# pengzhangzhi/ab_opt

Hardware: AMD Instinct MI355X
Metric: denoising steps/sec (256-res complex, 100-step sampler) (higher is better)
Workload: dtype f32

## Files before the change

### ab_opt_amd/csrc/ipa_core.hip

```cpp
#include <cstdlib>
#include "tail_common.h"
#include "kernels.h"

namespace abopt {

constexpr int NPW = 8, RPW = BI / NPW;
constexpr int NTH = 1024;
constexpr int SROW = 16 * JC + 4;
constexpr int SCLD = 17;
constexpr float kLog2e = 1.4426950408889634f;
constexpr float kSqrt13 = 0.5773502691896258f;
constexpr float kScale2 = kSqrt13 * kLog2e;
constexpr float kMask2 = 1e5f * kLog2e;
constexpr int SPLIT_ROW = H * C + H * D + H * P * 3;

__device__ __forceinline__ int sp_off(int h, int kq) { return h * JC + 4 * ((kq + (h >> 1)) & 3); }

__device__ __forceinline__ void point_local(float dx, float dy, float dz, float r0, float r1, float r2, float r3, float r4, float r5, float r6, float r7,
                                            float r8, float& lx, float& ly, float& lz, float& d, float& inv) {
    lx = __builtin_fmaf(r6, dz, __builtin_fmaf(r3, dy, r0 * dx));
    ly = __builtin_fmaf(r7, dz, __builtin_fmaf(r4, dy, r1 * dx));
    lz = __builtin_fmaf(r8, dz, __builtin_fmaf(r5, dy, r2 * dx));
    d = sqrtf(__builtin_fmaf(lz, lz, __builtin_fmaf(ly, ly, lx * lx)));
    inv = 1.f / (d + 1e-4f);
// ... 450 lines not shown
        sv_ += ringb[SLOT];                                                                                              \
        sv_ *= kScale2;                                                                                                  \
        float l2_[4];                                                                                                    \
        _Pragma("unroll") for (int r_ = 0; r_ < 4; ++r_) {                                                               \
            const float x_ = sv_[r_];                                                                                    \
            l2_[r_] = ((mk4_ >> (8 * r_)) & 0xffu) ? x_ : x_ - kMask2;                                                   \
        }                                                                                                                \
        const float mx_ = rows_max(fmaxf(fmaxf(l2_[0], l2_[1]), fmaxf(l2_[2], l2_[3])));                                 \
        const float mn_ = fmaxf(m_run[II], mx_);                                                                         \
        const float sc_ = __builtin_amdgcn_exp2f(m_run[II] - mn_);                                                       \
        f32x4 pv_;                                                                                                       \
        _Pragma("unroll") for (int r_ = 0; r_ < 4; ++r_) pv_[r_] = __builtin_amdgcn_exp2f(l2_[r_] - mn_);                \
        const float ps_ = rows_sum((pv_[0] + pv_[1]) + (pv_[2] + pv_[3]));                                               \
        l_run[II] = l_run[II] * sc_ + ps_;                                                                               \
        m_run[II] = mn_;                                                                                                 \
        _Pragma("unroll") for (int mt_ = 0; mt_ < 4; ++mt_) accP[II][mt_] *= sc_;                                        \
        _Pragma("unroll") for (int r_ = 0; r_ < 4; ++r_)                                                                 \
            _Pragma("unroll") for (int mt_ = 0; mt_ < 4; ++mt_) accP[II][mt_] = mfma4(ring[SLOT][r_][mt_], pv_[r_], accP[II][mt_]); \
        *reinterpret_cast<f32x4*>(spp_) = pv_;                                                                           \
        if (kq == 0) scl[((PAR) * BI + il_) * SCLD + fm] = sc_;                                                          \
    }
#define PP_CHUNK(K, CH, PAR)                                                                                             \
    {                                                                                                                    \
        const uint32_t mk4_ = *reinterpret_cast<const uint32_t*>(&mkc[(CH) * JC + kq * 4]);                              \
        PP_POS((2 * (K)) % 3, 0, CH, K, PAR)                                                                             \
        PP_POS((2 * (K) + 1) % 3, 1, CH, K, PAR)                                                                         \
    }
        int c = 0, j = 0;
        const uint8_t* mkc = mk;
        bool mi_b[RPW];
        auto block_begin = [&]() {
            if (j > 0) {
                bk = blk(j);
#pragma unroll
                for (int ii = 0; ii < RPW; ++ii) { zrow[ii] = zrow_n[ii]; pbrow[ii] = pbrow_n[ii]; }
            }
            has_next = j + 1 < nb;
            { const PBlk bn = blk(j + 1); rows_of(bn, zrow_n, pbrow_n); }
            mkc = mk + (j & 1) * mkld;
#pragma unroll
            for (int ii = 0; ii < RPW; ++ii) {
                mi_b[ii] = (bk.i0 + il0 + ii < L) && mkc[min(bk.i0 + il0 + ii, L - 1)] != 0;
                m_run[ii] = -INFINITY; l_run[ii] = 0.f;
#pragma unroll
                for (int mt = 0; mt < 4; ++mt) accP[ii][mt] = (f32x4){0.f, 0.f, 0.f, 0.f};
            }
        };
        auto block_end = [&]() {
#pragma unroll
            for (int ii = 0; ii < RPW; ++ii) {
                const int il = il0 + ii, i = bk.i0 + il;
                if (kq == 0) lsum[il * SCLD + fm] = l_run[ii];
                if (i < L && fm < H) {
                    const float inv = mi_b[ii] ? 1.f / l_run[ii] : 0.f;
                    float* fo = feat + (bk.rowbase + i) * FEAT + fm * C + kq * 16;
#pragma unroll
                    for (int r = 0; r < 4; ++r)
                        reinterpret_cast<f32x4*>(fo)[r] = (f32x4){accP[ii][0][r] * inv, accP[ii][1][r] * inv, accP[ii][2][r] * inv, accP[ii][3][r] * inv};
                }
            }
        };
#define PP_STEP(K, G)                                                                                                    \
    {                                                                                                                    \
        if (c == 0) block_begin();                                                                                       \
        PP_CHUNK(K, c, (G) & 1)                                                                                          \
        if (c == nchunk - 1) { block_end(); c = 0; ++j; } else ++c;                                                      \
        __syncthreads();                                                                                \
    }
        int g = 0;
        for (; g + 3 <= gtot; g += 3) { PP_STEP(0, g) PP_STEP(1, g + 1) PP_STEP(2, g + 2) }
        if (g < gtot) {
            PP_STEP(0, g)
            if (g + 1 < gtot) PP_STEP(1, g + 1)
        }
#undef PP_STEP
        __syncthreads();
    } else if (wave < NPW + 4) {
        const int h0 = (wave - NPW) * 3;
        const int atid = tid - NPW * 64;
        f32x4 kf[3][4];
        auto kv_of = [&](const PBlk& b) { return reinterpret_cast<const f32x4*>(kvfrag) + (int64_t)b.n * nchunk * H * 512; };
#define PA_ISSUE(HH, KV, CH) { const f32x4* fr_ = (KV) + ((int64_t)(CH) * H + h0 + (HH)) * 512 + lane;                   \
        _Pragma("unroll") for (int s_ = 0; s_ < 4; ++s_) kf[HH][s_] = fr_[s_ * 64]; }
        auto produce = [&](int buf, const f32x4* kv_next, int ch_next) {
#pragma unroll
            for (int hh = 0; hh < 3; ++hh) {
                const int h = h0 + hh;
                const f32x4* qh = qf + (h * 4) * 64 + lane;
                const f32x4 q0 = qh[0], q1 = qh[64], q2 = qh[128], q3 = qh[192];
                f32x4 acc0 = (f32x4){0.f, 0.f, 0.f, 0.f}, acc1 = acc0;
#pragma unroll
                for (int s = 0; s < 4; ++s) { acc0 = mfma4(kf[hh][0][s], q0[s], acc0); acc1 = mfma4(kf[hh][2][s], q2[s], acc1); }
#pragma unroll
                for (int s = 0; s < 4; ++s) { acc0 = mfma4(kf[hh][1][s], q1[s], acc0); if (s < 3) acc1 = mfma4(kf[hh][3][s], q3[s], acc1); }
                const f32x4 sres = acc0 + acc1;
                if (hh == 0) PA_ISSUE(0, kv_next, ch_next) else if (hh == 1) PA_ISSUE(1, kv_next, ch_next) else PA_ISSUE(2, kv_next, ch_next)
                *reinterpret_cast<f32x4*>(sp + (buf * BI + fm) * SROW + sp_off(h, kq)) = sres;
                __builtin_amdgcn_sched_barrier(0);
            }
        };
        auto kv_pos = [&](int p, const f32x4*& kv, int& ch) {
            const int pc = min(p, gtot - 1);
            const PBlk b = blk(pc / nchunk);
            kv = kv_of(b); ch = pc % nchunk;
        };
        {
            const f32x4* kv0; int ch0;
            kv_pos(0, kv0, ch0);
            PA_ISSUE(0, kv0, ch0) PA_ISSUE(1, kv0, ch0) PA_ISSUE(2, kv0, ch0)
        }
        fill_first();
        __syncthreads();
        { const f32x4* kv1; int ch1; kv_pos(1, kv1, ch1); produce(0, kv1, ch1); }
        __syncthreads();
        int bufn = 1;
        for (int g = 0; g < gtot; ++g) {
            const int gn = g + 1;
            if (gn < gtot) {
                if (gn % nchunk == 0) {
                    const int jn = gn / nchunk;
                    const PBlk bnx = blk(jn);
                    const f32x4* qg = reinterpret_cast<const f32x4*>(qfrag) + ((int64_t)bnx.n * nib + bnx.i0 / BI) * (H * 4 * 64);
#pragma unroll
                    for (int hh = 0; hh < 3; ++hh) {
                        f32x4 tq[4];
#pragma unroll
                        for (int s_ = 0; s_ < 4; ++s_) tq[s_] = qg[((h0 + hh) * 4 + s_) * 64 + lane];
#pragma unroll
                        for (int s_ = 0; s_ < 4; ++s_) qf[((h0 + hh) * 4 + s_) * 64 + lane] = tq[s_];
                    }
                    uint8_t* mkn = mk + (jn & 1) * mkld;
                    for (int e = atid; e < mkld; e += 4 * 64) mkn[e] = (e < L) ? mask[bnx.rowbase + e] : 0;
                    wave_lds_sync();
                }
                const f32x4* kvx; int chx;
                kv_pos(gn + 1, kvx, chx);
                produce(bufn, kvx, chx);
                bufn = (bufn == 2) ? 0 : bufn + 1;
            }
            if (g >= nchunk && g % nchunk == 1) {
                const PBlk bp = blk(g / nchunk - 1);
                persist_point_epilogue(ptsb, R, t, feat, bp.rowbase, bp.i0, L, atid, 4 * 64);
            }
            __syncthreads();
        }
        __syncthreads();
        { const PBlk bl = blk(nb - 1); persist_point_epilogue(ptsb, R, t, feat, bl.rowbase, bl.i0, L, atid, 4 * 64); }
    } else {
        const int h0 = (wave - NPW - 4) * 3;
        f32x4 vf[3][4];
        f32x4 accV[3][2], accT[3][2];
#pragma unroll
        for (int hh = 0; hh < 3; ++hh)
#pragma unroll
            for (int k = 0; k < 2; ++k) { accV[hh][k] = (f32x4){0.f, 0.f, 0.f, 0.f}; accT[hh][k] = (f32x4){0.f, 0.f, 0.f, 0.f}; }
        auto kv_of = [&](const PBlk& b) { return reinterpret_cast<const f32x4*>(kvfrag) + (int64_t)b.n * nchunk * H * 512; };
#define PC_ISSUE(HH, KV, CH) { const f32x4* fr_ = (KV) + ((int64_t)(CH) * H + h0 + (HH)) * 512 + 4 * 64 + lane;         \
        _Pragma("unroll") for (int s_ = 0; s_ < 4; ++s_) vf[HH][s_] = fr_[s_ * 64]; }
        auto kv_pos = [&](int p, const f32x4*& kv, int& ch) {
            const int pc = min(p, gtot - 1);
            const PBlk b = blk(pc / nchunk);
            kv = kv_of(b); ch = pc % nchunk;
        };
        auto consume = [&](int buf, int par, const f32x4* kv_next, int ch_next) {
#pragma unroll
            for (int hh = 0; hh < 3; ++hh) {
                const int h = h0 + hh;
                const float sc = scl[(par * BI + fm) * SCLD + h];
                const f32x4 pa = *reinterpret_cast<const f32x4*>(sp + (buf * BI + fm) * SROW + sp_off(h, kq));
                accV[hh][0] *= sc; accV[hh][1] *= sc; accT[hh][0] *= sc; accT[hh][1] *= sc;
#pragma unroll
                for (int s = 0; s < 4; ++s) {
                    accV[hh][0] = mfma4(vf[hh][s][0], pa[s], accV[hh][0]);
                    accV[hh][1] = mfma4(vf[hh][s][1], pa[s], accV[hh][1]);
                    accT[hh][0] = mfma4(vf[hh][s][2], pa[s], accT[hh][0]);
                    accT[hh][1] = mfma4(vf[hh][s][3], pa[s], accT[hh][1]);
                }
                if (hh == 0) PC_ISSUE(0, kv_next, ch_next) else if (hh == 1) PC_ISSUE(1, kv_next, ch_next) else PC_ISSUE(2, kv_next, ch_next)
                __builtin_amdgcn_sched_barrier(0);
            }
        };
        auto block_epilogue = [&](int j) {
            const PBlk b = blk(j);
            const uint8_t* mkc = mk + (j & 1) * mkld;
            const bool mi_c = (b.i0 + fm < L) && mkc[min(b.i0 + fm, L - 1)] != 0;
            const int i = b.i0 + fm;
#pragma unroll
            for (int hh = 0; hh < 3; ++hh) {
                const int h = h0 + hh;
                const float inv = mi_c ? 1.f / lsum[fm * SCLD + h] : 0.f;
                if (i < L) {
                    float* fo = feat + (b.rowbase + i) * FEAT + H * C + h * D + kq * 4;
                    *reinterpret_cast<f32x4*>(fo) = accV[hh][0] * inv;
                    *reinterpret_cast<f32x4*>(fo + 16) = accV[hh][1] * inv;
                }
                float* po = ptsb + (fm * H + h) * (P * 3) + kq * 3;
#pragma unroll
                for (int r = 0; r < 3; ++r) { po[r] = accT[hh][0][r] * inv; po[12 + r] = accT[hh][1][r] * inv; }
#pragma unroll
                for (int k = 0; k < 2; ++k) { accV[hh][k] = (f32x4){0.f, 0.f, 0.f, 0.f}; accT[hh][k] = (f32x4){0.f, 0.f, 0.f, 0.f}; }
            }
        };
        {
            const f32x4* kv0; int ch0;
            kv_pos(0, kv0, ch0);
            PC_ISSUE(0, kv0, ch0) PC_ISSUE(1, kv0, ch0) PC_ISSUE(2, kv0, ch0)
        }
        fill_first();
        __syncthreads();
        __syncthreads();
        __syncthreads();
        int buf = 0;
        for (int g = 1; g <= gtot; ++g) {
            const int p = g - 1;
            const f32x4* kvx; int chx;
            kv_pos(g, kvx, chx);
            consume(buf, p & 1, kvx, chx);
            buf = (buf == 2) ? 0 : buf + 1;
            if (p % nchunk == nchunk - 1) block_epilogue(p / nchunk);
            __syncthreads();
        }
    }
#undef PP_ISSUE
#undef PP_POS
#undef PP_CHUNK
#undef PA_ISSUE
#undef PC_ISSUE
}

constexpr int BI2 = 32, NPW2 = 4, RPW2 = BI2 / NPW2, NTH2 = 512, HPW = 6;

#define C32_L2(x, r) __builtin_fmaf((x), kScale2, mterm_[r])
__device__ long long g_clock_probe[2];
constexpr int PROF_SLOTS = 2048;
__device__ unsigned long long g_prof_span[PROF_SLOTS][2];
__global__ void prof_span_reset_kernel() {
    const int i = blockIdx.x * 256 + threadIdx.x;
    if (i < PROF_SLOTS) { g_prof_span[i][0] = ~0ull; g_prof_span[i][1] = 0ull; }
}
struct TailArgs {
    const float *wot, *wmf, *x, *ubias, *g1, *be1, *b0, *b1, *b2, *g2, *be2;
    float* out;
    unsigned* xt;
};
constexpr int C32_LOOP_LDS_FLOATS = 3 * 32 * SROW + 2 * 32 * SCLD + 32 * SCLD + 32 * 32;
constexpr int C32F_PTS_OFF = ((C32_LOOP_LDS_FLOATS * 4 + 2048 + 255) / 256) * 256;
constexpr int C32F_PTSLD = H * P * 3 + 4;
constexpr int C32F_LDS_BYTES = C32F_PTS_OFF + 32 * C32F_PTSLD * 4;
constexpr int C32F_U_OFF = 0, C32F_YS_OFF = MR * XLD * 4, C32F_APA_OFF = 2 * MR * XLD * 4;
constexpr int C32F_BIAS_OFF = 2 * OT_STAGE;
static_assert(2 * OT_STAGE <= 3 * 32 * SROW * 4, "staging buffers must fit into the S/P tile");
static_assert(C32F_BIAS_OFF + 3 * F * 4 <= 3 * 32 * SROW * 4 && C32F_APA_OFF + OT_NT * AP_PLANE <= 2 * OT_STAGE && OT_NT * AP_PLANE <= 32 * C32F_PTSLD * 4, "phase-2 buffers of the fused tail");
static_assert(C32F_LDS_BYTES <= 160 * 1024, "LDS of the fused block kernel");

__device__ __forceinline__ float mul_rn(float a, float b) {
#pragma clang fp contract(off)
    return a * b;
}
__device__ __forceinline__ void stage_put4(char* buf, int row, int col, float v0, float v1, float v2, float v3) {
    unsigned h0, l0, h1, l1;
    split_pair2(v0, v1, h0, l0);
    split_pair2(v2, v3, h1, l1);
    char* d = buf + row * OT_SROW + col * 2;
    *reinterpret_cast<uint2*>(d) = make_uint2(h0, h1);
    *reinterpret_cast<uint2*>(d + OT_PLANE) = make_uint2(l0, l1);
}

template <bool FUSE, bool ZT>
__global__ __launch_bounds__(NTH2) void ipa_core32_kernel(const float* __restrict__ qfrag, const float* __restrict__ kvfrag, const float* __restrict__ z,
                                                          const uint8_t* __restrict__ mask, const float* __restrict__ R, const float* __restrict__ t,
                                                          float* __restrict__ feat, const float* __restrict__ pbc, int L, int nib2, int xcd_remap, int z_shared,
                                                          TailArgs ta, int prof_slot, const float* __restrict__ zt, const float* __restrict__ zsc) {
    extern __shared__ __attribute__((aligned(16))) char smem_raw[];
    float* sp = reinterpret_cast<float*>(smem_raw);
    float* scl = sp + 3 * BI2 * SROW;
    float* lsum = scl + 2 * BI2 * SCLD;
    float* mlr = lsum + BI2 * SCLD;
    uint8_t* mk = reinterpret_cast<uint8_t*>(mlr + BI2 * 32);
    int n, ib;
    {
        const int b = blockIdx.x;
        if (xcd_remap == 2) {
            const int xcd = b & 7, k = b >> 3, per = nib2 * z_shared, r = k % per;
            ib = r / z_shared; n = (xcd + 8 * (k / per)) * z_shared + r % z_shared;
        } else if (xcd_remap) { const int xcd = b & 7, k = b >> 3; n = xcd + 8 * (k / nib2); ib = k % nib2; }
        else { n = b / nib2; ib = b % nib2; }
    }
    const int tid = threadIdx.x, lane = tid & 63, fm = lane & 15, kq = lane >> 4;
    const int wave = __builtin_amdgcn_readfirstlane(tid >> 6);
    const int nchunk = (L + JC - 1) / JC, nib16 = (L + BI - 1) / BI;
    const long long probe_c0 = clock64(), probe_w0 = wall_clock64();
    if (prof_slot >= 0 && threadIdx.x == 0) atomicMin(&g_prof_span[prof_slot][0], (unsigned long long)probe_w0);
    const int i0 = ib * BI2;
    const int64_t rowbase = (int64_t)n * L;
    const int64_t zbase = z_shared ? (int64_t)(n / z_shared) * L : rowbase;
    auto fill_mask = [&]() { for (int e = tid; e < nchunk * JC; e += NTH2) mk[e] = (e < L) ? mask[rowbase + e] : 0; };
    char* const stage = smem_raw;
    float* const ptsf = reinterpret_cast<float*>(smem_raw + C32F_PTS_OFF);
    const int64_t row0f = rowbase + i0, row_endf = rowbase + L;
    TailP2Pre<NTH2 / 64> pre;
    constexpr int RD = 12;
    struct WT { u32x4 h, l; };
    auto consumer = [&](int cb, WT (&wt)[RD]) {
        const u32x4* wfr = reinterpret_cast<const u32x4*>(ta.wot) + (int64_t)cb * OT_ST * OT_WVEC + lane;
        auto kstep = [&](int i) { return min(ot_chunk_at(min(i / OT_SPC, OT_NCH - 1)) * OT_SPC + (i % OT_SPC), OT_ST - 1); };
        f32x16 acc[4];
#pragma unroll
        for (int g = 0; g < 4; ++g) acc_zero(acc[g]);
        __syncthreads();
        const char* xrd = stage + (lane & 31) * OT_SROW + (lane >> 5) * 16;
#define C32F_KSTEP(P_, KK, NK)                                                                                           \
        {                                                                                                                \
            const int i_ = (P_) * OT_SPC + (KK);                                                                         \
            const u32x4 wH = wt[(KK) % RD].h, wL = wt[(KK) % RD].l;                                                      \
            const u32x4 xh = xnh, xl = xnl;                                                                              \
            if ((KK) + 1 < (NK)) {                                                                                       \
                xnh = *reinterpret_cast<const u32x4*>(xb + ((KK) % OT_SPC + 1) * 32); xnl = *reinterpret_cast<const u32x4*>(xb + ((KK) % OT_SPC + 1) * 32 + OT_PLANE); \
            }                                                                                                            \
            ot_kstep3(wH, wL, xh, xl, acc[((KK) % OT_SPC) / OT_SPW]);                                                    \
            if (i_ + RD < OT_ST) { const u32x4* nf_ = wfr + (int64_t)kstep(i_ + RD) * OT_WVEC; wt[(KK) % RD].h = nf_[0]; wt[(KK) % RD].l = nf_[64]; } \
        }
#define C32F_XFIRST() { xnh = *reinterpret_cast<const u32x4*>(xb); xnl = *reinterpret_cast<const u32x4*>(xb + OT_PLANE); }
        u32x4 xnh, xnl;
        static_assert(OT_SPC == 12 && OT_ST - (OT_NCH - 1) * OT_SPC == 6 && ot_chunk_at(OT_NCH - 1) == OT_NCH - 1, "positions 0..8 are full chunks, the last one holds six k-steps");
        static_assert((2 * OT_SPC) % RD == 0, "ring slots must repeat every two positions");
        for (int p = 0; p < OT_NCH - 2; p += 2) {
            {
                const char* xb = xrd;
                C32F_XFIRST()
                C32F_KSTEP(p, 0, 12) C32F_KSTEP(p, 1, 12) C32F_KSTEP(p, 2, 12) C32F_KSTEP(p, 3, 12) C32F_KSTEP(p, 4, 12) C32F_KSTEP(p, 5, 12)
                C32F_KSTEP(p, 6, 12) C32F_KSTEP(p, 7, 12) C32F_KSTEP(p, 8, 12) C32F_KSTEP(p, 9, 12) C32F_KSTEP(p, 10, 12) C32F_KSTEP(p, 11, 12)
                __syncthreads();
            }
            {
                const char* xb = xrd + OT_STAGE;
                C32F_XFIRST()
                C32F_KSTEP(p, 12, 24) C32F_KSTEP(p, 13, 24) C32F_KSTEP(p, 14, 24) C32F_KSTEP(p, 15, 24) C32F_KSTEP(p, 16, 24) C32F_KSTEP(p, 17, 24)
                C32F_KSTEP(p, 18, 24) C32F_KSTEP(p, 19, 24) C32F_KSTEP(p, 20, 24) C32F_KSTEP(p, 21, 24) C32F_KSTEP(p, 22, 24) C32F_KSTEP(p, 23, 24)
                __syncthreads();
            }
        }
        {
            const char* xb = xrd;
            C32F_XFIRST()
            C32F_KSTEP(8, 0, 12) C32F_KSTEP(8, 1, 12) C32F_KSTEP(8, 2, 12) C32F_KSTEP(8, 3, 12) C32F_KSTEP(8, 4, 12) C32F_KSTEP(8, 5, 12)
            C32F_KSTEP(8, 6, 12) C32F_KSTEP(8, 7, 12) C32F_KSTEP(8, 8, 12) C32F_KSTEP(8, 9, 12) C32F_KSTEP(8, 10, 12) C32F_KSTEP(8, 11, 12)
            __syncthreads();
        }
        {
            const char* xb = xrd + OT_STAGE;
            C32F_XFIRST()

            C32F_KSTEP(8, 12, 18) C32F_KSTEP(8, 13, 18) C32F_KSTEP(8, 14, 18) C32F_KSTEP(8, 15, 18) C32F_KSTEP(8, 16, 18) C32F_KSTEP(8, 17, 18)
            __syncthreads();
        }
#undef C32F_KSTEP
#undef C32F_XFIRST
        float (*us)[XLD] = reinterpret_cast<float (*)[XLD]>(smem_raw + C32F_U_OFF);
#pragma unroll
        for (int g = 0; g < 4; ++g) {
            f32x4 v;
#pragma unroll
            for (int e = 0; e < 4; ++e) {
                const int q = 4 * g + e;
                v[e] = (acc[0][q] + acc[1][q]) + (acc[2][q] + acc[3][q]);
            }
            *reinterpret_cast<f32x4*>(&us[lane & 31][cb * 32 + g * 8 + (lane >> 5) * 4]) = v;
        }
    };
    auto consumer_prefetch = [&](int cb, WT (&wt)[RD]) {
        const u32x4* wfr = reinterpret_cast<const u32x4*>(ta.wot) + (int64_t)cb * OT_ST * OT_WVEC + lane;
#pragma unroll
        for (int j = 0; j < RD; ++j) { const u32x4* f = wfr + (int64_t)(ot_chunk_at(0) * OT_SPC + j) * OT_WVEC; wt[j].h = f[0]; wt[j].l = f[64]; }
        static_assert(RD <= OT_SPC, "the first fragments belong to position 0");
    };

    if (wave < NPW2) {
        const int il0 = wave * RPW2;
        const int rows_tot_ = ((int)gridDim.x / nib2 / (z_shared ? z_shared : 1)) * L;
        const __amdgpu_buffer_rsrc_t zrs = ZT ? __builtin_amdgcn_make_buffer_rsrc(const_cast<float*>(zt), 0, (unsigned)rows_tot_ * (unsigned)nchunk * (JC * C * 4), 0x00020000)
                                              : __builtin_amdgcn_make_buffer_rsrc(const_cast<float*>(z + zbase * (int64_t)L * C), 0, L * L * C * 4, 0x00020000);
        const __amdgpu_buffer_rsrc_t brs = __builtin_amdgcn_make_buffer_rsrc(const_cast<float*>(pbc), 0, (unsigned)rows_tot_ * (unsigned)nchunk * (H * JC * 4), 0x00020000);
        int zrow[RPW2], pbrow[RPW2];
#pragma unroll
        for (int ii = 0; ii < RPW2; ++ii) {
            const int row = min(i0 + il0 + ii, L - 1);
            zrow[ii] = ZT ? ((int)zbase + row) * (JC * C * 4) : row * L * (C * 4);
            pbrow[ii] = ((int)zbase + row) * (H * JC * 4);
        }
        const unsigned lane_b = (unsigned)fm * 16u;
        const unsigned pb_lane = (unsigned)(min(fm, H - 1) * JC + kq * 4) * 4u;
        f32x4 ring[3][4], ringb[4];
        unsigned koff_[4], boff_;
#define P2_KOFF(CH)                                                                                                      \
    {                                                                                                                    \
        const int ch_ = min((CH), nchunk - 1);                                        \
        _Pragma("unroll") for (int r_ = 0; r_ < 4; ++r_) koff_[r_] = ZT ? ((unsigned)ch_ * (unsigned)(rows_tot_ * (JC * C * 4)) + (unsigned)(r_ * 1024 + lane * 16)) : (unsigned)min(ch_ * JC + kq * 4 + r_, L - 1) * (unsigned)(C * 4) + lane_b; \
    }
#define P2_BOFF(CH) boff_ = (unsigned)min((CH), nchunk - 1) * ((unsigned)rows_tot_ * (unsigned)(H * JC * 4)) + pb_lane;
#define P2_ISSUE_Z(SLOT, II)                                                                                            \
        _Pragma("unroll") for (int r_ = 0; r_ < 4; ++r_)                                                                \
            ring[SLOT][r_] = __builtin_bit_cast(f32x4, __builtin_amdgcn_raw_buffer_load_b128(zrs, koff_[r_], zrow[II], 2));
#define P2_ISSUE_B(SLOT, II) ringb[SLOT] = __builtin_bit_cast(f32x4, __builtin_amdgcn_raw_buffer_load_b128(brs, boff_, pbrow[II], 2));
        P2_KOFF(0) P2_BOFF(0)
        P2_ISSUE_B(0, 0) P2_ISSUE_Z(0, 0) P2_ISSUE_B(1, 1) P2_ISSUE_Z(1, 1) P2_ISSUE_B(2, 2)
        fill_mask();
        f32x4 accP[RPW2][4];
        float* mlw = mlr + (il0 * 16 + fm) * 2;
#pragma unroll
        for (int ii = 0; ii < RPW2; ++ii) {
            if (kq == 0) *reinterpret_cast<float2*>(mlw + ii * 32) = make_float2(-INFINITY, 0.f);
#pragma unroll
            for (int mt = 0; mt < 4; ++mt) accP[ii][mt] = (f32x4){0.f, 0.f, 0.f, 0.f};
        }
        const int spo = sp_off(fm, kq);
        __syncthreads();
        __syncthreads();
#define P2_SM(II, BUF)                                                                                                   \
    {                                                                                                                    \
        const int il_ = il0 + (II);                                                                                      \
        float* spp_ = sp + ((BUF) * BI2 + il_) * SROW + spo;                                                             \
        f32x4 sv_ = *reinterpret_cast<const f32x4*>(spp_);                                                               \
        const float2 ml_ = *reinterpret_cast<const float2*>(mlw + (II) * 32);                                            \
        sv_ += ringb[(II) & 3];                                                                                          \
        float l2_[4];                                                                                                    \
        _Pragma("unroll") for (int r_ = 0; r_ < 4; ++r_) l2_[r_] = C32_L2(sv_[r_], r_);          \
        const float mx_ = rows_max(fmaxf(fmaxf(l2_[0], l2_[1]), fmaxf(l2_[2], l2_[3])));                                 \
        const float mn_ = fmaxf(ml_.x, mx_);                                                                             \
        scn_ = __builtin_amdgcn_exp2f(ml_.x - mn_);                                                                      \
        _Pragma("unroll") for (int r_ = 0; r_ < 4; ++r_) pvn_[r_] = __builtin_amdgcn_exp2f(l2_[r_] - mn_);               \
        const float ps_ = rows_sum((pvn_[0] + pvn_[1]) + (pvn_[2] + pvn_[3]));                                           \
        const float ln_ = ml_.y * scn_ + ps_;                                                                            \
        *reinterpret_cast<f32x4*>(spp_) = pvn_;                                                                          \
        if (kq == 0) { scl[((CHPAR) * BI2 + il_) * SCLD + fm] = scn_; *reinterpret_cast<float2*>(mlw + (II) * 32) = make_float2(mn_, ln_); } \
    }
#define P2_MF(SLOT, II, K_)                                                                                              \
        accP[II][(K_) & 3] = mfma4(ring[SLOT][(K_) >> 2][(K_) & 3], pvc_[(K_) >> 2], accP[II][(K_) & 3]);                \
        __builtin_amdgcn_sched_barrier(0);
#define P2_POS(SLOT, II, CH, BUF)                                                                                        \
    {                                                                                                                    \
        const f32x4 pvc_ = pvn_;                                                                                         \
        if ((II) + 3 == 8) P2_BOFF((CH) + 1)                                 \
        if ((II) + 2 == 8) P2_KOFF((CH) + 1)                                                                             \
        P2_ISSUE_B(((II) + 3) & 3, ((II) + 3) & 7)                                                                       \
        P2_ISSUE_Z(((SLOT) + 2) % 3, ((II) + 2) & 7)                                                                     \
        const int il_ = il0 + (II) + 1;                                                                                  \
        float* spp_ = sp + ((BUF) * BI2 + il_) * SROW + spo;                                                             \
        f32x4 sv_ = *reinterpret_cast<const f32x4*>(spp_);                                                               \
        const float2 ml_ = *reinterpret_cast<const float2*>(mlw + ((II) + 1) * 32);                                      \
        __builtin_amdgcn_sched_barrier(0);                                                                               \
        P2_MF(SLOT, II, 0) P2_MF(SLOT, II, 1)                                                                            \
        sv_ += ringb[((II) + 1) & 3];                                                                                    \
        P2_MF(SLOT, II, 2)                                                                                               \
        float l2_[4];                                                                                                    \
        _Pragma("unroll") for (int r_ = 0; r_ < 4; ++r_) l2_[r_] = C32_L2(sv_[r_], r_);          \
        P2_MF(SLOT, II, 3)                                                                                               \
        float mx_ = fmaxf(fmaxf(l2_[0], l2_[1]), fmaxf(l2_[2], l2_[3]));                                                 \
        { auto a_ = __builtin_amdgcn_permlane16_swap(__float_as_uint(mx_), __float_as_uint(mx_), false, false);          \
          mx_ = fmaxf(__uint_as_float(a_[0]), __uint_as_float(a_[1])); }                                                 \
        P2_MF(SLOT, II, 4)                                                                                               \
        { auto b_ = __builtin_amdgcn_permlane32_swap(__float_as_uint(mx_), __float_as_uint(mx_), false, false);          \
          mx_ = fmaxf(__uint_as_float(b_[0]), __uint_as_float(b_[1])); }                                                 \
        const float mn_ = fmaxf(ml_.x, mx_);                                                                             \
        scn_ = __builtin_amdgcn_exp2f(ml_.x - mn_);                                                                      \
        P2_MF(SLOT, II, 5)                                                                                               \
        pvn_[0] = __builtin_amdgcn_exp2f(l2_[0] - mn_); pvn_[1] = __builtin_amdgcn_exp2f(l2_[1] - mn_); \
        P2_MF(SLOT, II, 6)                                                                                               \
        pvn_[2] = __builtin_amdgcn_exp2f(l2_[2] - mn_); pvn_[3] = __builtin_amdgcn_exp2f(l2_[3] - mn_); \
        float ps_ = (pvn_[0] + pvn_[1]) + (pvn_[2] + pvn_[3]);                                                           \
        P2_MF(SLOT, II, 7)                                                                                               \
        { auto a_ = __builtin_amdgcn_permlane16_swap(__float_as_uint(ps_), __float_as_uint(ps_), false, false);          \
          ps_ = __uint_as_float(a_[0]) + __uint_as_float(a_[1]); }                                                       \
        P2_MF(SLOT, II, 8)                                                                                               \
        { auto b_ = __builtin_amdgcn_permlane32_swap(__float_as_uint(ps_), __float_as_uint(ps_), false, false);          \
          ps_ = __uint_as_float(b_[0]) + __uint_as_float(b_[1]); }                                                       \
        const float ln_ = ml_.y * scn_ + ps_;                                                                            \
        P2_MF(SLOT, II, 9)                                                                                               \
        *reinterpret_cast<f32x4*>(spp_) = pvn_;                                                                          \
        P2_MF(SLOT, II, 10)                                                                                              \
        if (kq == 0) { scl[((CHPAR) * BI2 + il_) * SCLD + fm] = scn_; *reinterpret_cast<float2*>(mlw + ((II) + 1) * 32) = make_float2(mn_, ln_); } \
        __builtin_amdgcn_sched_barrier(0);                                                                               \
        P2_MF(SLOT, II, 11)                                                                                              \
        accP[(II) + 1][0] *= scn_;                                                                                       \
        P2_MF(SLOT, II, 12)                                                                                              \
        accP[(II) + 1][1] *= scn_;                                                                                       \
        P2_MF(SLOT, II, 13)                                                                                              \
        accP[(II) + 1][2] *= scn_;                                                                                       \
        P2_MF(SLOT, II, 14)                                                                                              \
        accP[(II) + 1][3] *= scn_;                                                                                       \
        P2_MF(SLOT, II, 15)                                                                                              \
    }
#define P2_POS_LAST(SLOT, II, CH)                                                                                        \
    {                                                                                                                    \
        const f32x4 pvc_ = pvn_;                                                                                         \
        if ((II) + 3 == 8) P2_BOFF((CH) + 1)                                 \
        if ((II) + 2 == 8) P2_KOFF((CH) + 1)                                                                             \
        P2_ISSUE_B(((II) + 3) & 3, ((II) + 3) & 7)                                                                       \
        P2_ISSUE_Z(((SLOT) + 2) % 3, ((II) + 2) & 7)                                                                     \
        _Pragma("unroll") for (int r_ = 0; r_ < 4; ++r_)                                                                 \
            _Pragma("unroll") for (int mt_ = 0; mt_ < 4; ++mt_) accP[II][mt_] = mfma4(ring[SLOT][r_][mt_], pvc_[r_], accP[II][mt_]); \
        __builtin_amdgcn_sched_barrier(0);                                                                               \
    }
#define P2H_SPLIT()                                                                                                      \
        { unsigned h01_, l01_, h23_, l23_;                                                                               \
          split_pair2(pvn_[0] * 16384.f, pvn_[1] * 16384.f, h01_, l01_); split_pair2(pvn_[2] * 16384.f, pvn_[3] * 16384.f, h23_, l23_); \
          pkn_ = (u32x4){h01_, h23_, l01_, l23_}; }
#define P2H_SM(II, BUF)                                                                                                   \
    {                                                                                                                    \
        const int il_ = il0 + (II);                                                                                      \
        float* spp_ = sp + ((BUF) * BI2 + il_) * SROW + spo;                                                             \
        f32x4 sv_ = *reinterpret_cast<const f32x4*>(spp_);                                                               \
        const float2 ml_ = *reinterpret_cast<const float2*>(mlw + (II) * 32);                                            \
        sv_ += ringb[(II) & 3];                                                                                          \
        float l2_[4];                                                                                                    \
        _Pragma("unroll") for (int r_ = 0; r_ < 4; ++r_) l2_[r_] = C32_L2(sv_[r_], r_);                                  \
        const float mx_ = rows_max(fmaxf(fmaxf(l2_[0], l2_[1]), fmaxf(l2_[2], l2_[3])));                                 \
        const float mn_ = fmaxf(ml_.x, mx_);                                                                             \
        scn_ = __builtin_amdgcn_exp2f(ml_.x - mn_);                                                                      \
        f32x4 pvn_;                                                                                                      \
        _Pragma("unroll") for (int r_ = 0; r_ < 4; ++r_) pvn_[r_] = __builtin_amdgcn_exp2f(l2_[r_] - mn_);               \
        const float ps_ = rows_sum((pvn_[0] + pvn_[1]) + (pvn_[2] + pvn_[3]));                                           \
        const float ln_ = ml_.y * scn_ + ps_;                                                                            \
        P2H_SPLIT()                                                                                                      \
        *reinterpret_cast<f32x4*>(spp_) = pvn_;                               \
        if (kq == 0) { scl[((CHPAR) * BI2 + il_) * SCLD + fm] = scn_; *reinterpret_cast<float2*>(mlw + (II) * 32) = make_float2(mn_, ln_); } \
    }
#define P2H_MF(SLOT, II, K_)                                                                                              \
        { const u32x4 za_ = __builtin_bit_cast(u32x4, ring[SLOT][(K_) & 3]);                                              \
          if ((K_) >> 2) accP[II][(K_) & 3] = mfma_h16((u32x2){za_[0], za_[1]}, bl_, accP[II][(K_) & 3]);                 \
          else accP[II][(K_) & 3] = mfma_h(za_, bh_, accP[II][(K_) & 3]); }                                              \
        __builtin_amdgcn_sched_barrier(0);
#define P2H_POS(SLOT, II, CH, BUF)                                                                                        \
    {                                                                                                                    \
        const u32x4 bh_ = (u32x4){pkn_[0], pkn_[1], pkn_[0], pkn_[1]}; const u32x2 bl_ = (u32x2){pkn_[2], pkn_[3]};          \
        if ((II) + 3 == 8) P2_BOFF((CH) + 1)                                 \
        if ((II) + 2 == 8) P2_KOFF((CH) + 1)                                                                             \
        P2_ISSUE_B(((II) + 3) & 3, ((II) + 3) & 7)                                                                       \
        P2_ISSUE_Z(((SLOT) + 2) % 3, ((II) + 2) & 7)                                                                     \
        const int il_ = il0 + (II) + 1;                                                                                  \
        float* spp_ = sp + ((BUF) * BI2 + il_) * SROW + spo;                                                             \
        f32x4 sv_ = *reinterpret_cast<const f32x4*>(spp_);                                                               \
        const float2 ml_ = *reinterpret_cast<const float2*>(mlw + ((II) + 1) * 32);                                      \
        __builtin_amdgcn_sched_barrier(0);                                                                               \
        P2H_MF(SLOT, II, 0) P2H_MF(SLOT, II, 1)                                                                            \
        sv_ += ringb[((II) + 1) & 3];                                                                                    \
        float l2_[4];                                                                                                    \
        _Pragma("unroll") for (int r_ = 0; r_ < 4; ++r_) l2_[r_] = C32_L2(sv_[r_], r_);                                  \
        P2H_MF(SLOT, II, 2)                                                                                               \
        float mx_ = fmaxf(fmaxf(l2_[0], l2_[1]), fmaxf(l2_[2], l2_[3]));                                                 \
        { auto a_ = __builtin_amdgcn_permlane16_swap(__float_as_uint(mx_), __float_as_uint(mx_), false, false);          \
          mx_ = fmaxf(__uint_as_float(a_[0]), __uint_as_float(a_[1])); }                                                 \
        P2H_MF(SLOT, II, 3)                                                                                               \
        { auto b_ = __builtin_amdgcn_permlane32_swap(__float_as_uint(mx_), __float_as_uint(mx_), false, false);          \
          mx_ = fmaxf(__uint_as_float(b_[0]), __uint_as_float(b_[1])); }                                                 \
        const float mn_ = fmaxf(ml_.x, mx_);                                                                             \
        scn_ = __builtin_amdgcn_exp2f(ml_.x - mn_);                                                                      \
        P2H_MF(SLOT, II, 4)                                                                                               \
        f32x4 pvn_;                                                                                                      \
        pvn_[0] = __builtin_amdgcn_exp2f(l2_[0] - mn_); pvn_[1] = __builtin_amdgcn_exp2f(l2_[1] - mn_); \
        pvn_[2] = __builtin_amdgcn_exp2f(l2_[2] - mn_); pvn_[3] = __builtin_amdgcn_exp2f(l2_[3] - mn_); \
        P2H_MF(SLOT, II, 5)                                                                                               \
        float ps_ = (pvn_[0] + pvn_[1]) + (pvn_[2] + pvn_[3]);                                                           \
        { auto a_ = __builtin_amdgcn_permlane16_swap(__float_as_uint(ps_), __float_as_uint(ps_), false, false);          \
          ps_ = __uint_as_float(a_[0]) + __uint_as_float(a_[1]); }                                                       \
        P2H_SPLIT()                                                                                                      \
        P2H_MF(SLOT, II, 6)                                                                                               \
        { auto b_ = __builtin_amdgcn_permlane32_swap(__float_as_uint(ps_), __float_as_uint(ps_), false, false);          \
          ps_ = __uint_as_float(b_[0]) + __uint_as_float(b_[1]); }                                                       \
        const float ln_ = ml_.y * scn_ + ps_;                                                                            \
        *reinterpret_cast<f32x4*>(spp_) = pvn_;                               \
        P2H_MF(SLOT, II, 7)                                                                                               \
        if (kq == 0) { scl[((CHPAR) * BI2 + il_) * SCLD + fm] = scn_; *reinterpret_cast<float2*>(mlw + ((II) + 1) * 32) = make_float2(mn_, ln_); } \
        __builtin_amdgcn_sched_barrier(0);                                                                               \
        if ((__builtin_amdgcn_ballot_w64(scn_ != 1.f) & 0x0fff0fff0fff0fffull) != 0ull) {                                \
            accP[(II) + 1][0] *= scn_; accP[(II) + 1][1] *= scn_; accP[(II) + 1][2] *= scn_; accP[(II) + 1][3] *= scn_; } \
    }
#define P2H_POS_LAST(SLOT, II, CH)                                                                                        \
    {                                                                                                                    \
        const u32x4 bh_ = (u32x4){pkn_[0], pkn_[1], pkn_[0], pkn_[1]}; const u32x2 bl_ = (u32x2){pkn_[2], pkn_[3]};          \
        if ((II) + 3 == 8) P2_BOFF((CH) + 1)                                                                             \
        if ((II) + 2 == 8) P2_KOFF((CH) + 1)                                                                             \
        P2_ISSUE_B(((II) + 3) & 3, ((II) + 3) & 7)                                                                       \
        P2_ISSUE_Z(((SLOT) + 2) % 3, ((II) + 2) & 7)                                                                     \
        P2H_MF(SLOT, II, 0) P2H_MF(SLOT, II, 1) P2H_MF(SLOT, II, 2) P2H_MF(SLOT, II, 3) P2H_MF(SLOT, II, 4) P2H_MF(SLOT, II, 5) P2H_MF(SLOT, II, 6) P2H_MF(SLOT, II, 7) \
    }
#define P2_SLOT(K, II) ((8 * (K) + (II)) % 3)
#define P2_CHUNK(K, CH)                                                                                                  \
    {                                                                                                                    \
        const uint32_t mk4_ = *reinterpret_cast<const uint32_t*>(&mk[(CH) * JC + kq * 4]);                               \
        float mterm_[4];                                                     \
        _Pragma("unroll") for (int r_ = 0; r_ < 4; ++r_) mterm_[r_] = ((mk4_ >> (8 * r_)) & 0xffu) ? 0.f : -kMask2;      \
        const int CHPAR = (CH) & 1;                                                                                      \
        f32x4 pvn_; float scn_;                                                                                                  \
        P2_SM(0, K)                                                                                                      \
        _Pragma("unroll") for (int mt_ = 0; mt_ < 4; ++mt_) accP[0][mt_] *= scn_;                                         \
        __builtin_amdgcn_sched_barrier(0);                                                                               \
        P2_POS(P2_SLOT(K, 0), 0, CH, K) P2_POS(P2_SLOT(K, 1), 1, CH, K) P2_POS(P2_SLOT(K, 2), 2, CH, K) P2_POS(P2_SLOT(K, 3), 3, CH, K) \
        P2_POS(P2_SLOT(K, 4), 4, CH, K) P2_POS(P2_SLOT(K, 5), 5, CH, K) P2_POS(P2_SLOT(K, 6), 6, CH, K) P2_POS_LAST(P2_SLOT(K, 7), 7, CH) \
        __syncthreads();                                                                          \
    }
#define P2H_CHUNK(K, CH)                                                                                                  \
    {                                                                                                                    \
        const uint32_t mk4_ = *reinterpret_cast<const uint32_t*>(&mk[(CH) * JC + kq * 4]);                               \
        float mterm_[4];                                                     \
        _Pragma("unroll") for (int r_ = 0; r_ < 4; ++r_) mterm_[r_] = ((mk4_ >> (8 * r_)) & 0xffu) ? 0.f : -kMask2;      \
        const int CHPAR = (CH) & 1;                                                                                      \
        u32x4 pkn_; float scn_;                                                                                                  \
        P2H_SM(0, K)                                                                                                      \
        _Pragma("unroll") for (int mt_ = 0; mt_ < 4; ++mt_) accP[0][mt_] *= scn_;                                         \
        __builtin_amdgcn_sched_barrier(0);                                                                               \
        P2H_POS(P2_SLOT(K, 0), 0, CH, K) P2H_POS(P2_SLOT(K, 1), 1, CH, K) P2H_POS(P2_SLOT(K, 2), 2, CH, K) P2H_POS(P2_SLOT(K, 3), 3, CH, K) \
        P2H_POS(P2_SLOT(K, 4), 4, CH, K) P2H_POS(P2_SLOT(K, 5), 5, CH, K) P2H_POS(P2_SLOT(K, 6), 6, CH, K) P2H_POS_LAST(P2_SLOT(K, 7), 7, CH) \
        __syncthreads();                                                                          \
    }
        int ch = 0;
        if constexpr (ZT) {
        for (; ch + 3 <= nchunk; ch += 3) { P2H_CHUNK(0, ch) P2H_CHUNK(1, ch + 1) P2H_CHUNK(2, ch + 2) }
        if (ch < nchunk) {
            P2H_CHUNK(0, ch)
            if (ch + 1 < nchunk) P2H_CHUNK(1, ch + 1)
        }
        } else {
        for (; ch + 3 <= nchunk; ch += 3) { P2_CHUNK(0, ch) P2_CHUNK(1, ch + 1) P2_CHUNK(2, ch + 2) }
        if (ch < nchunk) {
            P2_CHUNK(0, ch)
            if (ch + 1 < nchunk) P2_CHUNK(1, ch + 1)
        }
        }
#undef P2H_CHUNK
#undef P2H_POS
#undef P2H_POS_LAST
#undef P2H_MF
#undef P2H_SM
#undef P2H_SPLIT
#undef P2_CHUNK
#undef P2_SLOT
#undef P2_POS
#undef P2_POS_LAST
#undef P2_MF
#undef P2_SM
#undef P2_ISSUE_Z
#undef P2_ISSUE_B
#undef P2_KOFF
#undef P2_BOFF
        if constexpr (!FUSE) {
#pragma unroll
        for (int ii = 0; ii < RPW2; ++ii) {
            const int il = il0 + ii, i = i0 + il;
            const float l_fin = mlw[ii * 32 + 1];
            if (kq == 0) lsum[il * SCLD + fm] = l_fin;
            if (i < L && fm < H) {
                const bool mi = mk[i] != 0;
                const float inv = mi ? 1.f / l_fin : 0.f;
                float* fo = feat + (rowbase + i) * FEAT + fm * C + kq * 16;
#pragma unroll
                for (int r = 0; r < 4; ++r) {
                    if constexpr (ZT) {
                        const f32x4 zs = *reinterpret_cast<const f32x4*>(zsc + (zbase + i) * C + kq * 16 + r * 4);
                        reinterpret_cast<f32x4*>(fo)[r] = (f32x4){mul_rn(accP[ii][0][r], inv * zs[0]), mul_rn(accP[ii][1][r], inv * zs[1]), mul_rn(accP[ii][2][r], inv * zs[2]), mul_rn(accP[ii][3][r], inv * zs[3])};
                    } else
// ... 593 lines not shown
```

Before: 27800.

## Restructure output-projection consumer loop with buffer loads and deeper LDS prefetch

Replaces the macro-unrolled consumer k-step loop with a fully unrolled per-position loop. Weight fragments are now fetched through raw buffer loads using a buffer resource with constant offsets, replacing 64-bit pointer arithmetic. LDS activation reads use a three-deep register ring instead of two, and sched_barriers pin the issue order. The aim is lower address-computation overhead and better latency hiding, at the cost of more registers and constrained compiler scheduling.

```diff
diff --git a/ab_opt_amd/csrc/ipa_core.hip b/ab_opt_amd/csrc/ipa_core.hip
--- a/ab_opt_amd/csrc/ipa_core.hip
+++ b/ab_opt_amd/csrc/ipa_core.hip
@@ -776,60 +776,43 @@
     constexpr int RD = 12;
     struct WT { u32x4 h, l; };
     auto consumer = [&](int cb, WT (&wt)[RD]) {
-        const u32x4* wfr = reinterpret_cast<const u32x4*>(ta.wot) + (int64_t)cb * OT_ST * OT_WVEC + lane;
-        auto kstep = [&](int i) { return min(ot_chunk_at(min(i / OT_SPC, OT_NCH - 1)) * OT_SPC + (i % OT_SPC), OT_ST - 1); };
+        const __amdgpu_buffer_rsrc_t wrs = __builtin_amdgcn_make_buffer_rsrc(const_cast<float*>(ta.wot) + (int64_t)cb * OT_ST * OT_WVEC * 4, 0,
+                                                                             OT_ST * OT_WVEC * 16, 0x00020000);
+        const unsigned wlane = (unsigned)lane * 16u;
         f32x16 acc[4];
 #pragma unroll
         for (int g = 0; g < 4; ++g) acc_zero(acc[g]);
         __syncthreads();
         const char* xrd = stage + (lane & 31) * OT_SROW + (lane >> 5) * 16;
-#define C32F_KSTEP(P_, KK, NK)                                                                                           \
-        {                                                                                                                \
-            const int i_ = (P_) * OT_SPC + (KK);                                                                         \
-            const u32x4 wH = wt[(KK) % RD].h, wL = wt[(KK) % RD].l;                                                      \
-            const u32x4 xh = xnh, xl = xnl;                                                                              \
-            if ((KK) + 1 < (NK)) {                                                                                       \
-                xnh = *reinterpret_cast<const u32x4*>(xb + ((KK) % OT_SPC + 1) * 32); xnl = *reinterpret_cast<const u32x4*>(xb + ((KK) % OT_SPC + 1) * 32 + OT_PLANE); \
-            }                                                                                                            \
-            ot_kstep3(wH, wL, xh, xl, acc[((KK) % OT_SPC) / OT_SPW]);                                                    \
-            if (i_ + RD < OT_ST) { const u32x4* nf_ = wfr + (int64_t)kstep(i_ + RD) * OT_WVEC; wt[(KK) % RD].h = nf_[0]; wt[(KK) % RD].l = nf_[64]; } \
-        }
-#define C32F_XFIRST() { xnh = *reinterpret_cast<const u32x4*>(xb); xnl = *reinterpret_cast<const u32x4*>(xb + OT_PLANE); }
-        u32x4 xnh, xnl;
         static_assert(OT_SPC == 12 && OT_ST - (OT_NCH - 1) * OT_SPC == 6 && ot_chunk_at(OT_NCH - 1) == OT_NCH - 1, "positions 0..8 are full chunks, the last one holds six k-steps");
-        static_assert((2 * OT_SPC) % RD == 0, "ring slots must repeat every two positions");
-        for (int p = 0; p < OT_NCH - 2; p += 2) {
-            {
-                const char* xb = xrd;
-                C32F_XFIRST()
-                C32F_KSTEP(p, 0, 12) C32F_KSTEP(p, 1, 12) C32F_KSTEP(p, 2, 12) C32F_KSTEP(p, 3, 12) C32F_KSTEP(p, 4, 12) C32F_KSTEP(p, 5, 12)
-                C32F_KSTEP(p, 6, 12) C32F_KSTEP(p, 7, 12) C32F_KSTEP(p, 8, 12) C32F_KSTEP(p, 9, 12) C32F_KSTEP(p, 10, 12) C32F_KSTEP(p, 11, 12)
-                __syncthreads();
-            }
-            {
-                const char* xb = xrd + OT_STAGE;
-                C32F_XFIRST()
-                C32F_KSTEP(p, 12, 24) C32F_KSTEP(p, 13, 24) C32F_KSTEP(p, 14, 24) C32F_KSTEP(p, 15, 24) C32F_KSTEP(p, 16, 24) C32F_KSTEP(p, 17, 24)
-                C32F_KSTEP(p, 18, 24) C32F_KSTEP(p, 19, 24) C32F_KSTEP(p, 20, 24) C32F_KSTEP(p, 21, 24) C32F_KSTEP(p, 22, 24) C32F_KSTEP(p, 23, 24)
-                __syncthreads();
-            }
-        }
-        {
-            const char* xb = xrd;
-            C32F_XFIRST()
-            C32F_KSTEP(8, 0, 12) C32F_KSTEP(8, 1, 12) C32F_KSTEP(8, 2, 12) C32F_KSTEP(8, 3, 12) C32F_KSTEP(8, 4, 12) C32F_KSTEP(8, 5, 12)
-            C32F_KSTEP(8, 6, 12) C32F_KSTEP(8, 7, 12) C32F_KSTEP(8, 8, 12) C32F_KSTEP(8, 9, 12) C32F_KSTEP(8, 10, 12) C32F_KSTEP(8, 11, 12)
+        static_assert(RD == OT_SPC, "the ring slot of a k-step is its place in the position");
+#pragma unroll
+        for (int p = 0; p < OT_NCH; ++p) {
+            const int nk = p + 1 < OT_NCH ? OT_SPC : OT_ST - (OT_NCH - 1) * OT_SPC;
+            const char* xb = xrd + (p & 1) * OT_STAGE;
+            u32x4 xr[3][2];
+            xr[0][0] = *reinterpret_cast<const u32x4*>(xb); xr[0][1] = *reinterpret_cast<const u32x4*>(xb + OT_PLANE);
+            xr[1][0] = *reinterpret_cast<const u32x4*>(xb + 32); xr[1][1] = *reinterpret_cast<const u32x4*>(xb + 32 + OT_PLANE);
+            __builtin_amdgcn_sched_barrier(0);
+#pragma unroll
+            for (int kk = 0; kk < OT_SPC; ++kk) {
+                if (kk < nk) {
+                    const int i = p * OT_SPC + kk;
+                    if (kk + 2 < nk) {
+                        xr[(kk + 2) % 3][0] = *reinterpret_cast<const u32x4*>(xb + (kk + 2) * 32);
+                        xr[(kk + 2) % 3][1] = *reinterpret_cast<const u32x4*>(xb + (kk + 2) * 32 + OT_PLANE);
+                    }
+                    ot_kstep3(wt[kk].h, wt[kk].l, xr[kk % 3][0], xr[kk % 3][1], acc[kk / OT_SPW]);
+                    if (i + RD < OT_ST) {
+                        const unsigned wo = (unsigned)((ot_chunk_at((i + RD) / OT_SPC) * OT_SPC + (i + RD) % OT_SPC) * OT_WVEC * 16);
+                        wt[kk].h = __builtin_bit_cast(u32x4, __builtin_amdgcn_raw_buffer_load_b128(wrs, wlane, wo, 0));
+                        wt[kk].l = __builtin_bit_cast(u32x4, __builtin_amdgcn_raw_buffer_load_b128(wrs, wlane, wo + 64 * 16, 0));
+                    }
+                    __builtin_amdgcn_sched_barrier(0);
+                }
+            }
             __syncthreads();
         }
-        {
-            const char* xb = xrd + OT_STAGE;
-            C32F_XFIRST()
-
-            C32F_KSTEP(8, 12, 18) C32F_KSTEP(8, 13, 18) C32F_KSTEP(8, 14, 18) C32F_KSTEP(8, 15, 18) C32F_KSTEP(8, 16, 18) C32F_KSTEP(8, 17, 18)
-            __syncthreads();
-        }
-#undef C32F_KSTEP
-#undef C32F_XFIRST
         float (*us)[XLD] = reinterpret_cast<float (*)[XLD]>(smem_raw + C32F_U_OFF);
 #pragma unroll
         for (int g = 0; g < 4; ++g) {
```

After: 27910, median of 6. Within noise of the previous version (+0.4%).
